# batmanlab/Mammo-CLIP

Hardware: AMD Instinct MI355X
Metric: image-text pairs/s (whole node), EN-B5+BioClinicalBERT contrastive pre-training step (higher is better)
Workload: dtype bf16; 1 GPU; cfg4: efficientnet-b5 + BioClinicalBERT(BERT-base), 1024 pairs/GPU (2 views + 2 reports each), 1520x912 images, 256-token reports, breast_clip loss, AdamW; fwd+loss+bwd+optimizer; dropout/drop-connect on; global_batch=1024, parallelism=dp1 x 32 micro-batches, keep_graphs=7, recompute=0, keep_recompute=2, stat_tapes=True, streams=3

## Files before the change

include/mammoclip_hip.h:

```cpp
#ifndef MAMMOCLIP_HIP_H
#define MAMMOCLIP_HIP_H
#include <stdint.h>
#ifdef __cplusplus
extern "C" {
#endif

typedef uint16_t mc_bf16;

const char* mc_last_error(void);
int mc_version(void);
int mc_storage_is_f16(void);

typedef struct mc_gemm_args {
    const mc_bf16* A;
    const mc_bf16* B;
    void* C;
    long long M, K;
    int N;
    long long lda, ldb, ldc;
    int a_kmajor, b_kmajor;
    int c_f32, c_atomic;
    int splits;
    int batch, nb2;
    long long sA1, sA2, sB1, sB2, sC1, sC2;
// ... 154 lines not shown

typedef struct mc_bnact_args {
    const mc_bf16* x;
    long long n_img, hw;
    int c;
    const float* scale;
    const float* shift;
    int act;
    const float* rowscale;
    const mc_bf16* res;
    mc_bf16* out;
    float* pooled;
    const mc_bf16* g;
    const float* mul;
    const float* add;
    float add_scale;
    const float* mean;
    const float* invstd;
    float* partials;
    const float* coef;
    mc_bf16* dx;
    float* dgate;
    float* split_ws;
} mc_bnact_args;
int mc_bnact_rows(const mc_bnact_args* args);
int mc_bnact_img_splits(const mc_bnact_args* args);
int mc_bnact_apply(const mc_bnact_args* args, void* stream);
int mc_bnact_pool(const mc_bnact_args* args, void* stream);
int mc_bnact_bwd_reduce(const mc_bnact_args* args, void* stream);
int mc_bnact_bwd_apply(const mc_bnact_args* args, void* stream);
int mc_bnact_se_dgate(const mc_bnact_args* args, void* stream);
int mc_bnact_se_sums(const mc_bnact_args* args, void* stream);
int mc_bn_partials_from_se_sums(const float* sums, const float* gate, const float* dpooled, float add_scale,
                                long long n_img, int c, float* partials, void* stream);
int mc_bn_bwd_finalize(const float* partials, int rows, int c, double count, const float* gamma,
                       const float* mean, const float* invstd, float* dgamma, float* dbeta, float* coef,
                       void* stream);

int mc_bn_fold_prepare(const float* we, const float* coef, const float* xtx, const float* colsum_x, double rows, int n,
                       int k, mc_bf16* w1t, mc_bf16* wb, mc_bf16* sxx, void* stream);
int mc_bn_fold_cvec(const float* gt, const float* we, const float* coef, const float* dbeta, const float* colsum_x,
                    double rows, int n, int k, mc_bf16* gtb, float* cvec, void* stream);
int mc_bn_fold_wgrad(const float* t1, const float* wx, const float* coef, const float* dbeta, const float* colsum_x,
                     double rows, int n, int k, float* dwe, void* stream);
int mc_bn_gram_partials(const mc_bf16* w, int ldw, const float* xtx, const float* colsum_x, double rows, int n, int k,
                        float* partials, void* stream);

int mc_colsum_rows(long long m, int c);
int mc_colsum_bf16(const mc_bf16* x, long long m, int c, long long ld, float* partials, float* out,
                   int accumulate, void* stream);

int mc_se_fwd(const float* pooled, const float* w1, const float* b1, const float* w2, const float* b2,
              int n, int c, int cs, float* gate, float* ws , void* stream);
int mc_se_bwd(const float* pooled, const float* gate, const float* dgate, const float* w1, const float* b1,
              const float* w2, const float* b2, int n, int c, int cs, float* dpooled, float* dw1, float* db1,
              float* dw2, float* db2, float* ws, void* stream);

int mc_dropout_f32(const float* x, float* y, long long n, float p, unsigned long long seed,
                   unsigned int stream_id, void* stream);

int mc_bert_embed_fwd(const long long* ids, const long long* tt, const float* word, const float* pos,
                      const float* type, const float* gamma, const float* beta, float eps, int b, int t,
                      int h, float p, unsigned long long seed, unsigned int stream_id, mc_bf16* y,
                      float* mean, float* rstd, void* stream);
int mc_bert_embed_bwd(const mc_bf16* dy, const long long* ids, const long long* tt, const float* word,
                      const float* pos, const float* type, const float* gamma, const float* mean,
                      const float* rstd, int b, int t, int h, float p, unsigned long long seed,
                      unsigned int stream_id, float* dword, float* dpos, float* dtype, float* dgamma,
                      float* dbeta, void* stream);
// ... 106 lines not shown
```

mammo_clip_amd/breastclip/model/modules/efficientnet_custom.py:

```python
import math
from collections import namedtuple
from typing import List, Optional

import os

import torch
from torch import nn

from .... import ops

BN_MOMENTUM = 0.01
BN_EPS = 1e-3

VALID_MODELS = tuple(f"efficientnet-b{i}" for i in range(9)) + ("efficientnet-l2",)

_COEFFS = {
    "efficientnet-b0": (1.0, 1.0, 224, 0.2), "efficientnet-b1": (1.0, 1.1, 240, 0.2),
    "efficientnet-b2": (1.1, 1.2, 260, 0.3), "efficientnet-b3": (1.2, 1.4, 300, 0.3),
    "efficientnet-b4": (1.4, 1.8, 380, 0.4), "efficientnet-b5": (1.6, 2.2, 456, 0.4),
    "efficientnet-b6": (1.8, 2.6, 528, 0.5), "efficientnet-b7": (2.0, 3.1, 600, 0.5),
    "efficientnet-b8": (2.2, 3.6, 672, 0.5), "efficientnet-l2": (4.3, 5.3, 800, 0.5),
}
_STAGES = ((1, 3, 1, 1, 32, 16), (2, 3, 2, 6, 16, 24), (2, 5, 2, 6, 24, 40), (3, 3, 2, 6, 40, 80),
           (3, 5, 1, 6, 80, 112), (4, 5, 2, 6, 112, 192), (1, 3, 1, 6, 192, 320))
# ... 175 lines not shown
        n, h, wd, oh, ow, c0 = ctx.geo
        mod = ctx.mod
        link = ctx.link
        if link is not None:
            de, dgamma, dbeta = ops.bnact_bwd(e, n, oh * ow, c0, ctx.st, mod._bn0.weight, 0, g=dy.contiguous(), partials=link.part)
            link.part = None
        else:
            de, dgamma, dbeta = ops.bnact_bwd(e, n, oh * ow, c0, ctx.st, mod._bn0.weight, 1, g=dy.contiguous())
        l, r, t, b = mod.stem_pad
        patches = ops.stem_im2col(x, l, t, oh, ow)
        dw = ops.linear_wgrad(de, patches)
        gw, gg, gb = ops.deliver_param_grads((mod._conv_stem.weight, mod._bn0.weight, mod._bn0.bias),
                                             (dw[:, :27].reshape(c0, 3, 3, 3), dgamma, dbeta))
        return (None, gw, gg, gb, None) + ((None,) if link is not None else ())


class _StemLink:
    __slots__ = ("st", "part")

    def __init__(self):
        self.st, self.part = None, None


def _expand_conv(pl, x, we, stats=True):
    if pl.fp8_expand:
        return ops.linear_fwd_fp8(x, we, stats=True)
    return _conv_stats(ops.linear_fwd, pl.training, x, we, stats=stats)


def _depthwise(blk, pl, x, e, we, wkkc, pro0, stats=True):
    if pl.xdw:
        return _conv_stats(ops.mbconv_xdw_fwd, pl.training, x, we, pro0, wkkc, *pl.dw, stats=stats)
    return _conv_stats(ops.dwconv_fwd, pl.training, e if blk.args.expand != 1 else x, wkkc, *pl.dw, stats=stats, pro=pro0)


def _project_conv(pl, d, act1, st1, gate, wp, stats=True):
    ohw = pl.oh * pl.ow
    if pl.fp8_project:
        wg = ops.gate_weights(wp, gate)
        return ops.linear_fwd_fp8(act1, wg, stats=True, batch_w=(pl.n, ohw))
    src, pro = (act1, (None, None, gate, ohw)) if pl.keep_act else (d, (st1.scale, st1.shift, gate, ohw))
    return _conv_stats(ops.linear_fwd, pl.training, src, wp, stats=stats, pro=pro)


class _MBConvFn(torch.autograd.Function):

    @staticmethod
    def forward(ctx, x, rowscale, blk, n, h, w, recording, link, *params):
        a = blk.args
        pl = blk.plan(n, h, w, recording)
        training, ohw = pl.training, pl.oh * pl.ow
        wkkc = blk.w_taps()
        e = we = st0 = gram = None
        if a.expand != 1:
            we = blk.w_expand()
            if pl.xdw:
                if training and _replaying():
                    part0, gram = None, _TAPE.get()
                elif training:
                    part0, gram = ops.bn_gram_partials(x, we, n * h * w)
                    if _TAPE is not None:
                        _TAPE.put(gram)
                else:
                    part0 = None
            else:
                e, part0 = _expand_conv(pl, x, we)
            st0 = _bn_stats(part0, n * h * w, blk._bn0, training)
            pro0 = (st0.scale, st0.shift)
        else:
            pro0 = (link.st.scale, link.st.shift) if link is not None else None
        d, part1 = _depthwise(blk, pl, x, e, we, wkkc, pro0)
        st1 = _bn_stats(part1, n * ohw, blk._bn1, training)
        if pl.keep_act:
            pooled, act1 = ops.bnact_pool(d, n, ohw, a.cexp, st1.scale, st1.shift, 1, keep_act=True)
        elif training and _replaying():
            pooled, act1 = _TAPE.get(), None
        else:
            pooled, act1 = ops.bnact_pool(d, n, ohw, a.cexp, st1.scale, st1.shift, 1), None
            if training and _TAPE is not None:
                _TAPE.put(pooled)
        if training and _replaying():
            gate = _TAPE.get()
        else:
            gate = ops.se_fwd(pooled, blk._se_reduce.weight.view(a.cse, a.cexp), blk._se_reduce.bias,
                              blk._se_expand.weight.view(a.cexp, a.cse), blk._se_expand.bias)
            if training and _TAPE is not None:
                _TAPE.put(gate)
        wp = blk.w_project()
        p, part2 = _project_conv(pl, d, act1, st1, gate, wp)
        st2 = _bn_stats(part2, n * ohw, blk._bn2, training)
        y = ops.bnact_apply(p, n, ohw, a.cout, st2.scale, st2.shift, 0,
                            rowscale=rowscale if a.skip else None, res=x if a.skip else None)
        ctx.blk, ctx.plan, ctx.saved = blk, pl, dict(
            x=x, e=e if pl.store_e else None, d=d if pl.store_d else None, act1=act1 if pl.store_d else None,
            p=p if pl.store_p else None, we=we, wkkc=wkkc, wp=wp, pro0=pro0, link=link, st0=st0, st1=st1, st2=st2, gram=gram,
            pooled=pooled, gate=gate, efree=pl.efree, rowscale=rowscale if a.skip else None)
        return y

    @staticmethod
    def backward(ctx, dy):
        blk, pl, sv = ctx.blk, ctx.plan, ctx.saved
        a = blk.args
        n, h, w, oh, ow = pl.n, pl.h, pl.w, pl.oh, pl.ow
        hw, ohw = h * w, oh * ow
        k, s, l, t = a.k, a.s, a.pad[0], a.pad[2]
        dy = dy.contiguous()
        x, e, d, p, act1, link, pro0 = sv["x"], sv["e"], sv["d"], sv["p"], sv["act1"], sv["link"], sv["pro0"]
        st0, st1, st2, gate, pooled = sv["st0"], sv["st1"], sv["st2"], sv["gate"], sv["pooled"]
        if a.expand != 1 and e is None and not (pl.efree or pl.efree_s2):
            e = _expand_conv(pl, x, sv["we"], stats=False)[0]
        if d is None:
            d = _depthwise(blk, pl, x, e, sv["we"], sv["wkkc"], pro0, stats=False)[0]
            if pl.keep_act:
                act1 = ops.bnact_pool(d, n, ohw, a.cexp, st1.scale, st1.shift, 1, keep_act=True)[1]
        if p is None:
# ... 50 lines not shown
            da0 = ops.dwconv_bwd_data(dd, sv["wkkc"], *pl.dw, w_kkc_flipped=wflip)
            del dd
        if a.expand != 1:
            if de is not None:
                we_t = blk.w_expand(transposed=True)
                if pl.xbwd:
                    dx, dwe = ops.xbwd_rows(de, x, we_t, residual=dy if a.skip else None)
                else:
                    dx = ops.linear_dgrad(de, sv["we"], residual=dy if a.skip else None, w_t=we_t)
                    dwe = ops.linear_wgrad(de, x)
            grads["_expand_conv.weight"] = dwe.view(a.cexp, a.cin, 1, 1)
            grads["_bn0.weight"], grads["_bn0.bias"] = dg0, db0
        else:
            dx = da0
            if a.skip:
                dx = ops.bnact_apply(da0, n, hw, a.cin, blk._ones, blk._zeros, 0, res=dy)
        grads["_depthwise_conv.weight"] = ops.transpose_f32(dwdw).view(a.cexp, 1, k, k)
        grads["_bn1.weight"], grads["_bn1.bias"] = dg1, db1n
        grads["_se_reduce.weight"], grads["_se_reduce.bias"] = dw1.view(a.cse, a.cexp, 1, 1), db1
        grads["_se_expand.weight"], grads["_se_expand.bias"] = dw2.view(a.cexp, a.cse, 1, 1), dbse2
        grads["_project_conv.weight"] = dwp.view(a.cout, a.cexp, 1, 1)
        grads["_bn2.weight"], grads["_bn2.bias"] = dg2, db2
        ctx.saved = None
        return (dx, None, None, None, None, None, None, None) + ops.deliver_param_grads(blk._params(), [grads[nm] for nm in blk._param_names])


class _HeadFn(torch.autograd.Function):

    @staticmethod
    def forward(ctx, x, w, gamma, beta, mod, n, h, wd):
        cin, cout = w.shape[1], w.shape[0]
        wb = ops.cast_bf16(w.view(cout, cin))
        if mod.fp8 and cin % 16 == 0:
            e, part = ops.linear_fwd_fp8(x, wb, stats=True)
        else:
            e, part = _conv_stats(ops.linear_fwd, mod.training, x, wb)
        st = _bn_stats(part, n * h * wd, mod._bn1, mod.training)
        pooled = ops.bnact_pool(e, n, h * wd, cout, st.scale, st.shift, 1)
        ctx.mod, ctx.st, ctx.geo = mod, st, (n, h, wd, cin, cout)
        ctx.save_for_backward(x, e, wb)
        mod._head_cache = (e, st, n, h, wd, cout)
        return pooled

    @staticmethod
    def backward(ctx, dpooled):
        x, e, wb = ctx.saved_tensors
        n, h, wd, cin, cout = ctx.geo
# ... 114 lines not shown
    def w_taps(self, flipped=False):
        v = self._depthwise_conv.weight.view(self.args.cexp, self.args.k * self.args.k)
        return ops.flipped_taps_f32(v) if flipped else ops.transpose_f32(v, cache=True)

    def w_project(self, transposed=False):
        v = self._project_conv.weight.view(self.args.cout, self.args.cexp)
        return ops.cast_transpose_bf16(v) if transposed else ops.cast_bf16(v)

    def _params(self):
        cached = self.__dict__.get("_plist")
        if cached is not None:
            ps, slots = cached
            for p_, (d_, k_) in zip(ps, slots):
                if d_.get(k_) is not p_:
                    cached = None
                    break
        if cached is None:
            slots = [(m._parameters, k) for m in self.modules() for k, v in m._parameters.items() if v is not None]
            ps = [d_[k_] for d_, k_ in slots]
            assert len(ps) == len(self._param_names)
            self.__dict__["_plist"] = (ps, slots)
        return ps

    def forward(self, inputs, n, h, w, rowscale=None, link=None):
        return _MBConvFn.apply(inputs, rowscale, self, n, h, w, torch.is_grad_enabled(), link, *self._params())


class EfficientNet(nn.Module):

    def __init__(self, blocks_args: List[BlockArgs] = None, global_params: GlobalParams = None):
        super().__init__()
        assert isinstance(blocks_args, list) and len(blocks_args) > 0
        self._global_params, self._blocks_args = global_params, blocks_args
        gp = global_params
        size = (gp.image_size, gp.image_size) if isinstance(gp.image_size, int) else tuple(gp.image_size)
        c0 = _scaled_width(32, gp)
        self._conv_stem = _Conv(3, c0, 3, 2)
        self._bn0 = _BN(c0)
        self.stem_pad = _static_pad(size, 3, 2)
        size = _down(size, 2)
        self._blocks = nn.ModuleList([])
        for ba in blocks_args:
            ba = ba._replace(input_filters=_scaled_width(ba.input_filters, gp),
                             output_filters=_scaled_width(ba.output_filters, gp),
                             num_repeat=_scaled_depth(ba.num_repeat, gp))
            s = ba.stride if isinstance(ba.stride, int) else ba.stride[0]
            self._blocks.append(MBConvBlock(ba, gp, size, idx=len(self._blocks)))
            size = _down(size, s)
# ... 62 lines not shown

    def xdw_reforward_modes(self):
        changed = []
        for blk in self._blocks:
            if blk.recompute == 0 and blk.xdw_capable():
                changed.append((blk, blk.recompute))
                blk.recompute = 1
        return changed

    def set_swish(self, memory_efficient=True):
        """No-op: the swish is always the fused, recompute-in-backward form."""

    def stem_geo(self, n, h, w):
        l, r, t, b = self.stem_pad
        return n, _out_extent(h, t, b, 3, 2), _out_extent(w, l, r, 3, 2)

    def _stem(self, x):
        b0 = self._blocks[0].args
        link = _StemLink() if (LINK_STEM and b0.expand == 1 and not b0.skip and b0.s == 1) else None
        args = (x, self._conv_stem.weight, self._bn0.weight, self._bn0.bias, self)
        y = _StemFn.apply(*args, link) if link is not None else _StemFn.apply(*args)
        return y, link, self.stem_geo(x.shape[0], *x.shape[2:])

    def _drop_connect_scales(self, n, device, seed):
        rate = self._global_params.drop_connect_rate
        out = []
        nb = len(self._blocks)
        for i, blk in enumerate(self._blocks):
            p = rate * float(i) / nb if rate else 0.0
            if not (self.training and p > 0.0 and blk.args.skip):
                out.append(None)
                continue
            out.append(ops.dropout_f32(self._ones_b.expand(n).contiguous(), p, seed, 1000 + i))
        return out

    def _features_nhwc(self, inputs):
        if not inputs.is_cuda:
            raise RuntimeError("mammo_clip_amd.EfficientNet runs only on a HIP device (no CPU fallback)")
        x = inputs if isinstance(inputs, ops.RawImages) or inputs.dtype == torch.float32 else inputs.float()
        seed = self.rng.next()
        self._last_seed = seed
        counters = [] if self.training else None
        bns = self._bn_layers if counters is not None else ()
        for bn in bns:
            bn.defer_count = counters
        try:
            y, link, (n, h, w) = self._stem(x)
            scales = self._drop_connect_scales(n, x.device, seed)
            for blk, rs in zip(self._blocks, scales):
                y = blk(y, n, h, w, rs, link if blk.args.idx == 0 else None)
                n, h, w = blk.out_geo(n, h, w)
        finally:
            for bn in bns:
                bn.defer_count = None
        self._pending_counters = counters
        return y, n, h, w

    def warm_weight_images(self, backward: bool):
        for blk in self._blocks:
            if blk.args.expand != 1:
                blk.w_expand()
                if backward:
                    blk.w_expand(transposed=True)
            blk.w_taps()
            if backward and blk.args.s == 1:
                blk.w_taps(flipped=True)
            blk.w_project()
            if backward:
                blk.w_project(transposed=True)
        cout, cin = self._conv_head.weight.shape[0], self._conv_head.weight.shape[1]
        ops.cast_bf16(self._conv_head.weight.view(cout, cin))
        if backward:
            ops.cast_transpose_bf16(self._conv_head.weight.view(cout, cin))

# ... 25 lines not shown
            if torch.is_tensor(t_) and t_.is_cuda:
                t_.record_stream(side)
        seeds = [self.rng.next(), self.rng.next()]
        training = self.training
        counters = [[], []] if training else [None, None]
        bns = self._bn_layers if training else ()
        defer = None

        def chain(i):
            global _BN_DEFER
            torch.cuda.set_stream(side if i else main)
            for bn in bns:
                bn.defer_count = counters[i]
            _BN_DEFER = defer if i else None

        ys, scales, links = [None, None], [None, None], [None, None]
        try:
            torch.cuda.set_stream(side)
            defer = _BNDefer(self) if training else None
            for i in (0, 1):
                chain(i)
                ys[i], links[i], (n, h, w) = self._stem(xs[i])
                scales[i] = self._drop_connect_scales(n, xs[i].device, seeds[i])
            for bi, blk in enumerate(self._blocks):
                for i in (0, 1):
                    chain(i)
                    ys[i] = blk(ys[i], n, h, w, scales[i][bi], links[i] if bi == 0 else None)
                n, h, w = blk.out_geo(n, h, w)
            pooled = [None, None]
            for i in (0, 1):
                chain(i)
                pooled[i] = _HeadFn.apply(ys[i], self._conv_head.weight, self._bn1.weight, self._bn1.bias, self, n, h, w)
                if training and self._dropout_p > 0.0:
                    pooled[i] = _DropoutFn.apply(pooled[i], self._dropout_p, seeds[i], 999)
        finally:
            torch.cuda.set_stream(main)
            for bn in bns:
                bn.defer_count = None
            _BN_DEFER = None
        self._last_seed = seeds[1]
        main.wait_stream(side)
        if defer is not None:
            defer.apply()
        with torch.no_grad():
            for c in counters:
                if c:
                    torch._foreach_add_(c, 1)
        pooled[1].record_stream(main)
        return pooled[0], pooled[1]

    def _flush_counters(self):
# ... 30 lines not shown
```

mammo_clip_amd/csrc/bnact.hip:

```cpp
#include "common_hip.h"
#include "../../include/mammoclip_hip.h"

namespace {

__host__ __device__ inline int rowmap_width(int cv, int cbase, bool split_small) {
    if (cbase > 0) return (cv - cbase) < 256 ? (cv - cbase) : 256;
    if (cv > 256) return 256;
    if (!split_small || cv * (256 / cv) * 10 >= 256 * 7) return cv;
    int a = 1;
    while (a * 2 <= cv) a *= 2;
    return a;
}

struct RowMap {
    int cv, cvp, rpb, rl, cl;
    bool split_small;
    __device__ RowMap(int c, bool split_small_ = false) {
        cv = c / 8;
        split_small = split_small_;
        set(0);
    }
    __device__ void set(int cbase) {
        cvp = rowmap_width(cv, cbase, split_small);
        rpb = 256 / cvp;
// ... 52 lines not shown
    if (var < 0.0) var = 0.0;
    float is = (float)(1.0 / sqrt(var + (double)eps));
    mean[i] = (float)m;
    invstd[i] = is;
    float sc = gamma[i] * is;
    scale[i] = sc;
    shift[i] = beta[i] - (float)m * sc;
    if (update) {
        double unbiased = count > 1.0 ? var * count / (count - 1.0) : var;
        rmean[i] = (1.f - momentum) * rmean[i] + momentum * (float)m;
        rvar[i] = (1.f - momentum) * rvar[i] + momentum * (float)unbiased;
    }
}

__global__ void bn_eval_coeffs_k(const float* gamma, const float* beta, const float* rm, const float* rv, float eps,
                                 int c, float* scale, float* shift) {
    int i = blockIdx.x * blockDim.x + threadIdx.x;
    if (i >= c) return;
    float sc = gamma[i] / sqrtf(rv[i] + eps);
    scale[i] = sc;
    shift[i] = beta[i] - rm[i] * sc;
}

__global__ __launch_bounds__(256) void bnact_apply_k(const mc_bnact_args p) {
    const int cvn = p.c / 8;
    const long long total = p.n_img * p.hw * cvn;
    for (long long i = (long long)blockIdx.x * 256 + threadIdx.x; i < total; i += (long long)gridDim.x * 256) {
        int cv = (int)(i % cvn);
        long long pix = i / cvn;
        float f[8], s[8], t[8];
        unpack8(nt_load16(p.x + pix * p.c + cv * 8), f);
        load8f(p.scale + cv * 8, s);
        load8f(p.shift + cv * 8, t);
        float rs = p.rowscale ? p.rowscale[pix / p.hw] : 1.f;
        if (p.act == 1) bn_silu8(f, s, t);
        else {
#pragma unroll
            for (int q = 0; q < 8; ++q) f[q] = f[q] * s[q] + t[q];
        }
#pragma unroll
        for (int q = 0; q < 8; ++q) f[q] *= rs;
        if (p.res) {
            float r[8];
            unpack8(nt_load16(p.res + pix * p.c + cv * 8), r);
#pragma unroll
            for (int q = 0; q < 8; ++q) f[q] += r[q];
        }
        *reinterpret_cast<uint4*>(p.out + pix * p.c + cv * 8) = pack8(f);
    }
}

template <int MODE>
__global__ __launch_bounds__(256) void bnact_img_reduce_k(const mc_bnact_args p) {
    RowMap rm(p.c, MODE == 0);
    __shared__ float red[256 * 8];
    __shared__ float tmp[256];
    const long long img = blockIdx.x;
    const bf16_t* xb = p.x + img * p.hw * p.c;
    const bf16_t* gb = (MODE == 1) ? p.g + img * p.hw * p.c : nullptr;
    float* dst = (MODE == 0 ? p.pooled : p.dgate) + img * p.c;
    const float post = (MODE == 0) ? 1.0f / (float)p.hw : 1.0f;
    for (int cbase = 0; cbase < rm.cv; cbase += rm.cvp) {
        rm.set(cbase);
        int v = cbase + rm.cl;
        float acc[8];
#pragma unroll
        for (int q = 0; q < 8; ++q) acc[q] = 0.f;
        if (rm.rl < rm.rpb && v < rm.cv) {
            float s[8], t[8];
            load8f(p.scale + v * 8, s);
            load8f(p.shift + v * 8, t);
// ... 457 lines not shown
                       gamma, beta, running_mean, running_var, momentum, eps, update_running, mean, invstd, scale, shift);
    MC_LAUNCH_CHECK();
    return MC_OK;
}
extern "C" int mc_bn_eval_coeffs(const float* gamma, const float* beta, const float* running_mean,
                                 const float* running_var, float eps, int c, float* scale, float* shift, void* stream) {
    MC_CHECK(gamma && beta && running_mean && running_var && scale && shift && c > 0, "bn_eval_coeffs: bad args");
    hipLaunchKernelGGL(bn_eval_coeffs_k, dim3(mc_div_up(c, 128)), dim3(128), 0, (hipStream_t)stream, gamma, beta,
                       running_mean, running_var, eps, c, scale, shift);
    MC_LAUNCH_CHECK();
    return MC_OK;
}
static int bwd_grid_x(const mc_bnact_args& p) {
    int cv = p.c / 8;
    int cvp = rowmap_width(cv, 0, false);
    int rpb = 256 / (cvp > 0 ? cvp : 1);
    long long per = (p.hw + (long long)rpb * 32 - 1) / ((long long)rpb * 32);
    long long cap = 4096 / (p.n_img > 0 ? p.n_img : 1);
    if (cap < 1) cap = 1;
    long long gx = per < cap ? per : cap;
    return (int)(gx < 1 ? 1 : gx);
}
extern "C" int mc_bnact_rows(const mc_bnact_args* a) { return (int)(bwd_grid_x(*a) * a->n_img); }
extern "C" int mc_bnact_apply(const mc_bnact_args* a, void* stream) {
    const mc_bnact_args& p = *a;
    if (int e = check_bnact(p)) return e;
    MC_CHECK(p.out, "bnact_apply: null out");
    hipLaunchKernelGGL(bnact_apply_k, dim3(stream_blocks(p.n_img * p.hw * (p.c / 8))), dim3(256), 0, (hipStream_t)stream, p);
    MC_LAUNCH_CHECK();
    return MC_OK;
}
__global__ __launch_bounds__(256) void split_sum_k(const float* __restrict__ ws, float* __restrict__ out, long long n, int splits) {
    __shared__ float sh[4][64];
    const int el = threadIdx.x & 63, pl = threadIdx.x >> 6;
    const long long i = (long long)blockIdx.x * 64 + el;
    float s = 0.f;
    if (i < n) {
        int k = pl;
        for (; k + 12 < splits; k += 16) {
            const float a = ws[(long long)k * n + i], b = ws[(long long)(k + 4) * n + i];
            const float c = ws[(long long)(k + 8) * n + i], d = ws[(long long)(k + 12) * n + i];
            s += a; s += b; s += c; s += d;
        }
        for (; k < splits; k += 4) s += ws[(long long)k * n + i];
    }
    sh[pl][el] = s;
    __syncthreads();
    if (pl == 0 && i < n) out[i] = ((sh[0][el] + sh[1][el]) + sh[2][el]) + sh[3][el];
}
static int img_splits(const mc_bnact_args& p, long long target = 2048) {
// ... 126 lines not shown
```

mammo_clip_amd/csrc/bnfold.hip:

```cpp
#include "common_hip.h"
#include "../../include/mammoclip_hip.h"

namespace {

#ifdef MC_F16
#define MC_FOLD_ROWS(rows) (rows)
#else
#define MC_FOLD_ROWS(rows) 1.0
#endif
__global__ void fold_prepare_k(const float* __restrict__ we, const float* __restrict__ coef, const float* __restrict__ xtx,
                               const float* __restrict__ cs, double rows, int n, int k, bf16_t* __restrict__ w1t,
                               bf16_t* __restrict__ wb, bf16_t* __restrict__ sxx) {
    const long long nk = (long long)n * k, total = nk + (long long)k * k;
    for (long long idx = (long long)blockIdx.x * 256 + threadIdx.x; idx < total; idx += (long long)gridDim.x * 256) {
        if (idx < nk) {
            const int i = (int)(idx / k), j = (int)(idx % k);
            const float w = we[idx];
            w1t[(long long)j * n + i] = f2bf(w * coef[i]);
            wb[idx] = f2bf((float)((double)(w * coef[n + i]) * MC_FOLD_ROWS(rows)));
        } else {
            const long long r = idx - nk;
            const int i = (int)(r / k), j = (int)(r % k);
            sxx[r] = f2bf((float)(((double)xtx[r] - (double)cs[i] * (double)cs[j] / rows) / MC_FOLD_ROWS(rows)));
        }
// ... 43 lines not shown
    for (int idx = threadIdx.x; idx < k * k; idx += 256) {
        const int i = idx / k, j = idx - i * k;
        const double sij = (double)xtx[idx] - (double)cs[i] * (double)cs[j] / rows;
        q += (double)bf2f(wc[i]) * sij * (double)bf2f(wc[j]);
    }
    __shared__ double red[2][256];
    red[0][threadIdx.x] = s; red[1][threadIdx.x] = q;
    __syncthreads();
    for (int st = 128; st > 0; st >>= 1) {
        if (threadIdx.x < st) { red[0][threadIdx.x] += red[0][threadIdx.x + st]; red[1][threadIdx.x] += red[1][threadIdx.x + st]; }
        __syncthreads();
    }
    if (threadIdx.x == 0) {
        const double sum = red[0][0];
        double sq = red[1][0];
        if (sq < 0.0) sq = 0.0;
        sq += sum * sum / rows;
        const float s_hi = (float)sum, q_hi = (float)sq;
        part[c] = s_hi; part[n + c] = q_hi;
        part[2 * n + c] = (float)(sum - (double)s_hi); part[3 * n + c] = (float)(sq - (double)q_hi);
    }
}

}

extern "C" int mc_bn_gram_partials(const mc_bf16* w, int ldw, const float* xtx, const float* colsum_x, double rows, int n, int k,
                                   float* partials, void* stream) {
    MC_CHECK(w && xtx && colsum_x && partials && n > 0 && k > 0 && ldw >= k && rows > 0, "bn_gram_partials: bad args");
    hipLaunchKernelGGL(gram_partials_k, dim3(n), dim3(256), 0, (hipStream_t)stream, (const bf16_t*)w, ldw, xtx, colsum_x, rows, n, k,
                       partials);
    MC_LAUNCH_CHECK();
    return MC_OK;
}

extern "C" int mc_bn_fold_prepare(const float* we, const float* coef, const float* xtx, const float* colsum_x, double rows,
                                  int n, int k, mc_bf16* w1t, mc_bf16* wb, mc_bf16* sxx, void* stream) {
    MC_CHECK(we && coef && xtx && colsum_x && w1t && wb && sxx && n > 0 && k > 0 && rows > 0, "bn_fold_prepare: bad args");
    const long long total = (long long)n * k + (long long)k * k;
    hipLaunchKernelGGL(fold_prepare_k, dim3((unsigned)((total + 255) / 256 < 2048 ? (total + 255) / 256 : 2048)), dim3(256), 0,
                       (hipStream_t)stream, we, coef, xtx, colsum_x, rows, n, k, (bf16_t*)w1t, (bf16_t*)wb, (bf16_t*)sxx);
    MC_LAUNCH_CHECK();
    return MC_OK;
}

extern "C" int mc_bn_fold_cvec(const float* gt, const float* we, const float* coef, const float* dbeta,
                               const float* colsum_x, double rows, int n, int k, mc_bf16* gtb, float* cvec, void* stream) {
// ... 17 lines not shown
```

mammo_clip_amd/lib.py:

```python
import ctypes as C
import os

_HERE = os.path.dirname(os.path.abspath(__file__))
STORAGE = os.environ.get("MC_STORAGE", "bf16").lower()
if STORAGE not in ("bf16", "f16"):
    raise ValueError(f"MC_STORAGE must be 'bf16' or 'f16', got {STORAGE!r}")
LIB_PATH = os.path.join(_HERE, "lib", "libmammoclip_hip.so" if STORAGE == "bf16" else "libmammoclip_hip_f16.so")

P, LL, I, F, D, U, ULL = C.c_void_p, C.c_longlong, C.c_int, C.c_float, C.c_double, C.c_uint, C.c_ulonglong


class GemmArgs(C.Structure):
    _fields_ = [
        ("A", P), ("B", P), ("C", P),
        ("M", LL), ("K", LL), ("N", I),
        ("lda", LL), ("ldb", LL), ("ldc", LL),
        ("a_kmajor", I), ("b_kmajor", I),
        ("c_f32", I), ("c_atomic", I),
        ("splits", I),
        ("batch", I), ("nb2", I),
        ("sA1", LL), ("sA2", LL), ("sB1", LL), ("sB2", LL), ("sC1", LL), ("sC2", LL),
        ("bias", P), ("bias_stride1", LL),
        ("act", I),
        ("R", P), ("ldr", LL),
# ... 33 lines not shown
    ]


class DwconvArgs(C.Structure):
    _fields_ = [
        ("x", P), ("dy", P), ("out", P), ("w_kkc", P),
        ("n", I), ("h", I), ("w", I), ("c", I),
        ("k", I), ("stride", I), ("pad_l", I), ("pad_t", I), ("oh", I), ("ow", I),
        ("pro_scale", P), ("pro_shift", P), ("stat_partials", P),
        ("epi_x", P), ("epi_scale", P), ("epi_shift", P), ("epi_mean", P), ("epi_invstd", P),
        ("dw_out", P), ("stat_rows", I),
        ("xw", P), ("cin", I),
    ]


class BnactArgs(C.Structure):
    _fields_ = [
        ("x", P), ("n_img", LL), ("hw", LL), ("c", I),
        ("scale", P), ("shift", P), ("act", I),
        ("rowscale", P), ("res", P), ("out", P),
        ("pooled", P),
        ("g", P), ("mul", P), ("add", P), ("add_scale", F), ("mean", P), ("invstd", P),
        ("partials", P), ("coef", P), ("dx", P), ("dgate", P), ("split_ws", P),
    ]


class AdamwTensor(C.Structure):
    _fields_ = [("param", P), ("grad", P), ("exp_avg", P), ("exp_avg_sq", P), ("numel", LL), ("bf16_image", P)]


_SIGS = {
    "mc_version": ([], I),
    "mc_storage_is_f16": ([], I),
    "mc_adamw_step": ([C.POINTER(AdamwTensor), I, D, D, D, D, D, LL, P], I),
    "mc_grads_unscale": ([C.POINTER(AdamwTensor), I, F, P, P], I),
    "mc_grads_unscale_dev": ([C.POINTER(AdamwTensor), I, P, P, P], I),
    "mc_adamw_step_ls": ([C.POINTER(AdamwTensor), I, D, D, D, D, D, LL, P, P, P], I),
    "mc_loss_scale_update": ([P, P, D, D, I, I, P], I),
    "mc_grad_norm_partials": ([C.POINTER(AdamwTensor), I], LL),
    "mc_grad_norm": ([C.POINTER(AdamwTensor), I, P, LL, F, P, P], I),
    "mc_grads_unscale_norm_dev": ([C.POINTER(AdamwTensor), I, P, P, P, LL, F, P, P], I),
    "mc_grads_scale_dev": ([C.POINTER(AdamwTensor), I, P, P], I),
    "mc_adamw_step_clip": ([C.POINTER(AdamwTensor), I, D, D, D, D, D, LL, P, P, P, P], I),
    "mc_gemm_bf16": ([C.POINTER(GemmArgs), P], I),
    "mc_gemm_stat_rows": ([C.POINTER(GemmArgs)], I),
    "mc_gemm_tile_config": ([C.POINTER(GemmArgs)], I),
# ... 20 lines not shown
    "mc_stem_weight_prep": ([P, P, I, P], I),
    "mc_stem_im2col": ([P, LL, LL, LL, LL, I, I, I, I, I, I, I, P, P], I),
    "mc_image_minmax_u8": ([P, LL, LL, I, P, P], I),
    "mc_gate_weights_bf16": ([P, P, I, I, I, P, P], I),
    "mc_stem_im2col_u8": ([P, LL, LL, LL, LL, P, F, F, I, I, I, I, I, I, I, P, P], I),
    "mc_dwconv_stat_rows": ([C.POINTER(DwconvArgs)], I),
    "mc_dwconv_bwd_data_stat_rows": ([C.POINTER(DwconvArgs)], I),
    "mc_dwconv_fwd": ([C.POINTER(DwconvArgs), P], I),
    "mc_dwconv_bwd_data": ([C.POINTER(DwconvArgs), P], I),
    "mc_dwconv_bwd_data_xw_supported": ([C.POINTER(DwconvArgs)], I),
    "mc_dwconv_bwd_data_plan": ([C.POINTER(DwconvArgs), C.POINTER(C.c_int)], I),
    "mc_dwconv_bwd_data_xw_preferred": ([C.POINTER(DwconvArgs)], I),
    "mc_dwconv_bwd_weight": ([C.POINTER(DwconvArgs), P], I),
    "mc_dwconv_set_lane_mode": ([I], I),
    "mc_dwconv_lane_supported": ([C.POINTER(DwconvArgs)], I),
    "mc_dwconv_bwd_fused_supported": ([C.POINTER(DwconvArgs)], I),
    "mc_dwconv_bwd_fused_preferred": ([C.POINTER(DwconvArgs)], I),
    "mc_dwconv_bwd_fused_stat_rows": ([C.POINTER(DwconvArgs)], I),
    "mc_dwconv_bwd_fused": ([C.POINTER(DwconvArgs), P], I),
    "mc_mbconv_xdw_supported": ([C.POINTER(DwconvArgs)], I),
    "mc_mbconv_xdw_stat_rows": ([C.POINTER(DwconvArgs)], I),
    "mc_mbconv_xdw_fwd": ([C.POINTER(DwconvArgs), P], I),
    "mc_bn_gram_partials": ([P, I, P, P, D, I, I, P, P], I),
    "mc_bn_finalize": ([P, I, I, D, P, P, P, P, F, F, I, P, P, P, P, P], I),
    "mc_bn_eval_coeffs": ([P, P, P, P, F, I, P, P, P], I),
    "mc_bnact_rows": ([C.POINTER(BnactArgs)], I),
    "mc_bnact_img_splits": ([C.POINTER(BnactArgs)], I),
    "mc_bnact_apply": ([C.POINTER(BnactArgs), P], I),
    "mc_bnact_pool": ([C.POINTER(BnactArgs), P], I),
    "mc_bnact_bwd_reduce": ([C.POINTER(BnactArgs), P], I),
    "mc_bnact_bwd_apply": ([C.POINTER(BnactArgs), P], I),
    "mc_bnact_se_dgate": ([C.POINTER(BnactArgs), P], I),
    "mc_bnact_se_sums": ([C.POINTER(BnactArgs), P], I),
    "mc_bn_partials_from_se_sums": ([P, P, P, F, LL, I, P, P], I),
    "mc_bn_bwd_finalize": ([P, I, I, D, P, P, P, P, P, P, P], I),
    "mc_colsum_rows": ([LL, I], I),
    "mc_colsum_bf16": ([P, LL, I, LL, P, P, I, P], I),
    "mc_se_fwd": ([P, P, P, P, P, I, I, I, P, P, P], I),
    "mc_se_bwd": ([P, P, P, P, P, P, P, I, I, I, P, P, P, P, P, P, P], I),
    "mc_dropout_f32": ([P, P, LL, F, ULL, U, P], I),
    "mc_bert_embed_fwd": ([P, P, P, P, P, P, P, F, I, I, I, F, ULL, U, P, P, P, P], I),
    "mc_bert_embed_bwd": ([P, P, P, P, P, P, P, P, P, I, I, I, F, ULL, U, P, P, P, P, P, P], I),
    "mc_add_ln_fwd": ([P, P, P, P, F, LL, I, F, ULL, U, P, P, P, P], I),
    "mc_add_ln_bwd": ([P, P, P, P, P, P, LL, I, F, ULL, U, P, P, P, P, P], I),
    "mc_softmax_fwd": ([P, LL, I, F, ULL, U, P, P, P], I),
    "mc_softmax_bwd": ([P, P, LL, I, F, ULL, U, F, P, P], I),
    "mc_bn_fold_prepare": ([P, P, P, P, D, I, I, P, P, P, P], I),
    "mc_bn_fold_cvec": ([P, P, P, P, P, D, I, I, P, P, P], I),
    "mc_bn_fold_wgrad": ([P, P, P, P, P, D, I, I, P, P], I),
# ... 117 lines not shown
```

mammo_clip_amd/ops.py:

```python
import ctypes as C
import math
import os

import weakref

import torch

from . import lib as L

BF16 = torch.bfloat16 if L.STORAGE == "bf16" else torch.float16


def _p(t):
    return None if t is None else t.data_ptr()


_RAW_STREAM = getattr(torch._C, "_cuda_getCurrentRawStream", None)
_GET_DEV = getattr(torch._C, "_cuda_getDevice", None)


def _st():
    if _RAW_STREAM is None or _GET_DEV is None:
        return torch.cuda.current_stream().cuda_stream
    return _RAW_STREAM(_GET_DEV())
# ... 653 lines not shown
        a = _dw_args(n, h, w, c, k, stride, pad_l, pad_t, oh, ow)
        a.cin = cin
        hit = _XDW_OK[key] = bool(L.load().mc_mbconv_xdw_supported(C.byref(a)))
    return hit


def mbconv_xdw_fwd(x, we, pro, w_kkc, n, h, w, c, k, stride, pad_l, pad_t, oh, ow, stats=False):
    cin = x.shape[1]
    assert we.shape == (c, cin) and we.is_contiguous() and x.is_contiguous()
    a = _dw_args(n, h, w, c, k, stride, pad_l, pad_t, oh, ow)
    y = empty((n * oh * ow, c), BF16, x)
    a.x, a.out, a.w_kkc, a.xw, a.cin = _p(x), _p(y), _p(w_kkc), _p(we), cin
    a.pro_scale, a.pro_shift = _p(pro[0]), _p(pro[1])
    part = None
    if stats:
        rows = L.load().mc_mbconv_xdw_stat_rows(C.byref(a))
        part = empty((rows, 2, c), torch.float32, x)
        a.stat_partials, a.stat_rows = _p(part), rows
    _note(2 * n * (cin * h * w + c * oh * ow) + 2 * c * cin, 2 * n * c * (oh * ow * k * k + h * w * cin))
    L.call("mc_mbconv_xdw_fwd", C.byref(a), _st(), kind=f"k{k}s{stride}")
    return (y, part) if stats else y


def bn_gram_partials(x, we, rows):
    c, cin = we.shape
    xtx = linear_wgrad(x, x, tag="_xtx")
    cs = colsum(x)
    part = empty((2, 2, c), torch.float32, x)
    L.call("mc_bn_gram_partials", _p(we), we.stride(0), _p(xtx), _p(cs), float(rows), c, cin, _p(part), _st())
    return part, (xtx, cs)


def _dwconv_bwd_weight_impl(x, dy, n, h, w, c, k, stride, pad_l, pad_t, oh, ow, pro=None):
    a = _dw_args(n, h, w, c, k, stride, pad_l, pad_t, oh, ow)
    dw = torch.zeros((k * k, c), dtype=torch.float32, device=x.device)
    a.x, a.dy, a.out = _p(x), _p(dy), _p(dw)
    if pro is not None:
        a.pro_scale, a.pro_shift = _p(pro[0]), _p(pro[1])
    _note(2 * n * c * (h * w + oh * ow), 2 * n * c * oh * ow * k * k)
    L.call("mc_dwconv_bwd_weight", C.byref(a), _st(), kind=f"k{k}s{stride}")
    return dw


class BNStats:
    __slots__ = ("mean", "invstd", "scale", "shift", "count")


def bn_finalize(partials, count, gamma, beta, running_mean, running_var, momentum, eps, update_running):
    rows, _, c = partials.shape
    buf = empty((4, c), torch.float32, partials)
    L.call("mc_bn_finalize", _p(partials), rows, c, float(count), _p(gamma), _p(beta), _p(running_mean),
           _p(running_var), momentum, eps, int(update_running), _p(buf[0]), _p(buf[1]), _p(buf[2]), _p(buf[3]), _st())
    s = BNStats()
    s.mean, s.invstd, s.scale, s.shift, s.count = buf[0], buf[1], buf[2], buf[3], float(count)
    return s


def bn_eval_coeffs(gamma, beta, running_mean, running_var, eps):
    c = gamma.shape[0]
    buf = empty((4, c), torch.float32, gamma)
    L.call("mc_bn_eval_coeffs", _p(gamma), _p(beta), _p(running_mean), _p(running_var), eps, c, _p(buf[2]), _p(buf[3]), _st())
    s = BNStats()
    s.mean, s.invstd, s.scale, s.shift, s.count = None, None, buf[2], buf[3], 0.0
    return s


def _bnact(x, n_img, hw, c, scale, shift, act):
    a = L.BnactArgs()
    a.x, a.n_img, a.hw, a.c = _p(x), n_img, hw, c
    a.scale, a.shift, a.act = _p(scale), _p(shift), act
    return a


def bnact_apply(x, n_img, hw, c, scale, shift, act, rowscale=None, res=None):
    a = _bnact(x, n_img, hw, c, scale, shift, act)
    out = empty((n_img * hw, c), BF16, x)
    a.rowscale, a.res, a.out = _p(rowscale), _p(res), _p(out)
    _note(2 * n_img * hw * c * (3 if res is not None else 2))
    L.call("mc_bnact_apply", C.byref(a), _st())
    return out


def _split_ws(a, x, n_img, c, planes=1):
    sp = L.load().mc_bnact_img_splits(C.byref(a))
    if sp <= 1:
        return None
    ws = empty((sp, planes, n_img, c), torch.float32, x)
    a.split_ws = _p(ws)
    return ws


def bnact_pool(x, n_img, hw, c, scale, shift, act, keep_act=False):
    a = _bnact(x, n_img, hw, c, scale, shift, act)
    pooled = empty((n_img, c), torch.float32, x)
    a.pooled = _p(pooled)
    y = None
    if keep_act:
        y = empty((n_img * hw, c), BF16, x)
        a.out = _p(y)
    ws = _split_ws(a, x, n_img, c)
    _note((4 if keep_act else 2) * n_img * hw * c)
    L.call("mc_bnact_pool", C.byref(a), _st())
    return (pooled, y) if keep_act else pooled
# ... 683 lines not shown
```

Baseline: 125.3 image-text pairs/s.

## Fuse next block's Gram matrix and column sums into the BN-apply epilogue

When the next MBConv block takes the xdw path, which needs X^T X and colsum(X) of its input for BN statistics, the current block's bnact_apply now computes these in the same pass with an MFMA-based Gram epilogue. The result is passed to the next block through a link object. This removes a separate re-read of the activation (the linear_wgrad xtx GEMM plus the colsum kernel) for narrow channel counts (c <= 64). It adds a new kernel whose per-block partials need an extra combine launch and workspace, and the Gram matrix is now accumulated from bf16-rounded outputs.

After: 126.4 image-text pairs/s, median of 6. No clear change (+0.8%).

```diff
diff --git a/include/mammoclip_hip.h b/include/mammoclip_hip.h
--- a/include/mammoclip_hip.h
+++ b/include/mammoclip_hip.h
@@ -200,8 +200,12 @@
     mc_bf16* dx;
     float* dgate;
     float* split_ws;
+    float* gram_ws;
+    float* gram_xtx;
+    float* gram_colsum;
 } mc_bnact_args;
 int mc_bnact_rows(const mc_bnact_args* args);
+int mc_bnact_gram_parts(const mc_bnact_args* args);
 int mc_bnact_img_splits(const mc_bnact_args* args);
 int mc_bnact_apply(const mc_bnact_args* args, void* stream);
 int mc_bnact_pool(const mc_bnact_args* args, void* stream);
@@ -223,6 +227,7 @@
                      double rows, int n, int k, float* dwe, void* stream);
 int mc_bn_gram_partials(const mc_bf16* w, int ldw, const float* xtx, const float* colsum_x, double rows, int n, int k,
                         float* partials, void* stream);
+int mc_bn_gram_combine(const float* ws, int parts, int k, float* xtx, float* colsum_x, void* stream);
 
 int mc_colsum_rows(long long m, int c);
 int mc_colsum_bf16(const mc_bf16* x, long long m, int c, long long ld, float* partials, float* out,
diff --git a/mammo_clip_amd/breastclip/model/modules/efficientnet_custom.py b/mammo_clip_amd/breastclip/model/modules/efficientnet_custom.py
--- a/mammo_clip_amd/breastclip/model/modules/efficientnet_custom.py
+++ b/mammo_clip_amd/breastclip/model/modules/efficientnet_custom.py
@@ -221,6 +221,18 @@
         self.st, self.part = None, None
 
 
+class _GramLink:
+    __slots__ = ("want", "pair", "ptr")
+
+    def __init__(self):
+        self.want, self.pair, self.ptr = False, None, 0
+
+    def take(self, x):
+        pair, ptr = self.pair, self.ptr
+        self.pair, self.ptr = None, 0
+        return pair if (pair is not None and ptr == x.data_ptr()) else None
+
+
 def _expand_conv(pl, x, we, stats=True):
     if pl.fp8_expand:
         return ops.linear_fwd_fp8(x, we, stats=True)
@@ -245,7 +257,7 @@
 class _MBConvFn(torch.autograd.Function):
 
     @staticmethod
-    def forward(ctx, x, rowscale, blk, n, h, w, recording, link, *params):
+    def forward(ctx, x, rowscale, blk, n, h, w, recording, link, glink, *params):
         a = blk.args
         pl = blk.plan(n, h, w, recording)
         training, ohw = pl.training, pl.oh * pl.ow
@@ -257,7 +269,7 @@
                 if training and _replaying():
                     part0, gram = None, _TAPE.get()
                 elif training:
-                    part0, gram = ops.bn_gram_partials(x, we, n * h * w)
+                    part0, gram = ops.bn_gram_partials(x, we, n * h * w, gram=glink.take(x) if glink is not None else None)
                     if _TAPE is not None:
                         _TAPE.put(gram)
                 else:
@@ -288,8 +300,12 @@
         wp = blk.w_project()
         p, part2 = _project_conv(pl, d, act1, st1, gate, wp)
         st2 = _bn_stats(part2, n * ohw, blk._bn2, training)
+        want = glink is not None and glink.want and training and not _replaying() and ops.bnact_gram_ok(a.cout)
         y = ops.bnact_apply(p, n, ohw, a.cout, st2.scale, st2.shift, 0,
-                            rowscale=rowscale if a.skip else None, res=x if a.skip else None)
+                            rowscale=rowscale if a.skip else None, res=x if a.skip else None, gram=want)
+        if want:
+            y, glink.pair = y
+            glink.ptr = y.data_ptr()
         ctx.blk, ctx.plan, ctx.saved = blk, pl, dict(
             x=x, e=e if pl.store_e else None, d=d if pl.store_d else None, act1=act1 if pl.store_d else None,
             p=p if pl.store_p else None, we=we, wkkc=wkkc, wp=wp, pro0=pro0, link=link, st0=st0, st1=st1, st2=st2, gram=gram,
@@ -386,7 +402,7 @@
         grads["_project_conv.weight"] = dwp.view(a.cout, a.cexp, 1, 1)
         grads["_bn2.weight"], grads["_bn2.bias"] = dg2, db2
         ctx.saved = None
-        return (dx, None, None, None, None, None, None, None) + ops.deliver_param_grads(blk._params(), [grads[nm] for nm in blk._param_names])
+        return (dx, None, None, None, None, None, None, None, None) + ops.deliver_param_grads(blk._params(), [grads[nm] for nm in blk._param_names])
 
 
 class _HeadFn(torch.autograd.Function):
@@ -547,8 +563,12 @@
             self.__dict__["_plist"] = (ps, slots)
         return ps
 
-    def forward(self, inputs, n, h, w, rowscale=None, link=None):
-        return _MBConvFn.apply(inputs, rowscale, self, n, h, w, torch.is_grad_enabled(), link, *self._params())
+    def forward(self, inputs, n, h, w, rowscale=None, link=None, glink=None):
+        return _MBConvFn.apply(inputs, rowscale, self, n, h, w, torch.is_grad_enabled(), link, glink, *self._params())
+
+    def wants_gram(self, n, h, w):
+        return (self.training and self.xdw_capable() and ops.bnact_gram_ok(self.args.cin)
+                and self.plan(n, h, w, torch.is_grad_enabled()).xdw)
 
 
 class EfficientNet(nn.Module):
@@ -657,6 +677,13 @@
         y = _StemFn.apply(*args, link) if link is not None else _StemFn.apply(*args)
         return y, link, self.stem_geo(x.shape[0], *x.shape[2:])
 
+    def _gram_link(self):
+        if not (ops.GRAM_PRODUCER and self.training) or _replaying():
+            return None
+        if any(blk._forward_hooks or blk._forward_pre_hooks for blk in self._blocks):
+            return None
+        return _GramLink()
+
     def _drop_connect_scales(self, n, device, seed):
         rate = self._global_params.drop_connect_rate
         out = []
@@ -682,9 +709,13 @@
         try:
             y, link, (n, h, w) = self._stem(x)
             scales = self._drop_connect_scales(n, x.device, seed)
-            for blk, rs in zip(self._blocks, scales):
-                y = blk(y, n, h, w, rs, link if blk.args.idx == 0 else None)
-                n, h, w = blk.out_geo(n, h, w)
+            glink = self._gram_link()
+            for bi, (blk, rs) in enumerate(zip(self._blocks, scales)):
+                geo = blk.out_geo(n, h, w)
+                if glink is not None:
+                    glink.want = bi + 1 < len(self._blocks) and self._blocks[bi + 1].wants_gram(*geo)
+                y = blk(y, n, h, w, rs, link if blk.args.idx == 0 else None, glink)
+                n, h, w = geo
         finally:
             for bn in bns:
                 bn.defer_count = None
@@ -756,11 +787,16 @@
                 chain(i)
                 ys[i], links[i], (n, h, w) = self._stem(xs[i])
                 scales[i] = self._drop_connect_scales(n, xs[i].device, seeds[i])
+            glinks = [self._gram_link(), self._gram_link()]
             for bi, blk in enumerate(self._blocks):
+                geo = blk.out_geo(n, h, w)
+                want = glinks[0] is not None and bi + 1 < len(self._blocks) and self._blocks[bi + 1].wants_gram(*geo)
                 for i in (0, 1):
                     chain(i)
-                    ys[i] = blk(ys[i], n, h, w, scales[i][bi], links[i] if bi == 0 else None)
-                n, h, w = blk.out_geo(n, h, w)
+                    if glinks[i] is not None:
+                        glinks[i].want = want
+                    ys[i] = blk(ys[i], n, h, w, scales[i][bi], links[i] if bi == 0 else None, glinks[i])
+                n, h, w = geo
             pooled = [None, None]
             for i in (0, 1):
                 chain(i)
diff --git a/mammo_clip_amd/csrc/bnact.hip b/mammo_clip_amd/csrc/bnact.hip
--- a/mammo_clip_amd/csrc/bnact.hip
+++ b/mammo_clip_amd/csrc/bnact.hip
@@ -98,31 +98,160 @@
     shift[i] = beta[i] - rm[i] * sc;
 }
 
+__device__ __forceinline__ uint4 bnact_apply8(const uint4& xv, const float* s, const float* t, int act, float rs, bool has_res,
+                                              const uint4& rv) {
+    float f[8];
+    unpack8(xv, f);
+    if (act == 1) bn_silu8(f, s, t);
+    else {
+#pragma unroll
+        for (int q = 0; q < 8; ++q) f[q] = __builtin_fmaf(f[q], s[q], t[q]);
+    }
+#pragma unroll
+    for (int q = 0; q < 8; ++q) {
+        f[q] *= rs;
+        asm volatile("" : "+v"(f[q]));
+    }
+    if (has_res) {
+        float r[8];
+        unpack8(rv, r);
+#pragma unroll
+        for (int q = 0; q < 8; ++q) f[q] += r[q];
+    }
+    return pack8(f);
+}
+
 __global__ __launch_bounds__(256) void bnact_apply_k(const mc_bnact_args p) {
     const int cvn = p.c / 8;
     const long long total = p.n_img * p.hw * cvn;
     for (long long i = (long long)blockIdx.x * 256 + threadIdx.x; i < total; i += (long long)gridDim.x * 256) {
         int cv = (int)(i % cvn);
         long long pix = i / cvn;
-        float f[8], s[8], t[8];
-        unpack8(nt_load16(p.x + pix * p.c + cv * 8), f);
+        float s[8], t[8];
+        const uint4 xv = nt_load16(p.x + pix * p.c + cv * 8);
         load8f(p.scale + cv * 8, s);
         load8f(p.shift + cv * 8, t);
         float rs = p.rowscale ? p.rowscale[pix / p.hw] : 1.f;
-        if (p.act == 1) bn_silu8(f, s, t);
-        else {
-#pragma unroll
-            for (int q = 0; q < 8; ++q) f[q] = f[q] * s[q] + t[q];
-        }
-#pragma unroll
-        for (int q = 0; q < 8; ++q) f[q] *= rs;
-        if (p.res) {
-            float r[8];
-            unpack8(nt_load16(p.res + pix * p.c + cv * 8), r);
-#pragma unroll
-            for (int q = 0; q < 8; ++q) f[q] += r[q];
-        }
-        *reinterpret_cast<uint4*>(p.out + pix * p.c + cv * 8) = pack8(f);
+        const uint4 rv = p.res ? nt_load16(p.res + pix * p.c + cv * 8) : make_uint4(0u, 0u, 0u, 0u);
+        *reinterpret_cast<uint4*>(p.out + pix * p.c + cv * 8) = bnact_apply8(xv, s, t, p.act, rs, p.res != nullptr, rv);
+    }
+}
+
+typedef __attribute__((ext_vector_type(4))) short s4_t;
+typedef __attribute__((address_space(3))) s4_t lds_s4_t;
+__device__ __forceinline__ bf16x8_t tr_frag(const unsigned char* tile, int rs, int row0, int col0, int lane) {
+    const int g = lane >> 4, i = lane & 15;
+    const unsigned char* a = tile + (size_t)(row0 + g * 8 + (i >> 2)) * rs + (col0 + (i & 3) * 4) * 2;
+    s4_t lo = __builtin_amdgcn_ds_read_tr16_b64_v4i16((lds_s4_t*)(a));
+    s4_t hi = __builtin_amdgcn_ds_read_tr16_b64_v4i16((lds_s4_t*)(a + 4 * rs));
+    typedef __attribute__((ext_vector_type(8))) short s8_t;
+    s8_t v = {lo[0], lo[1], lo[2], lo[3], hi[0], hi[1], hi[2], hi[3]};
+    return __builtin_bit_cast(bf16x8_t, v);
+}
+
+constexpr int GRAM_WROWS = 64;
+constexpr int GRAM_SROWS = 4 * GRAM_WROWS;
+constexpr int GRAM_MAX_PARTS = 512;
+
+template <int CV>
+__global__ __launch_bounds__(256, 2) void bnact_apply_gram_k(const mc_bnact_args p) {
+    constexpr int C = CV * 8, NF = (C + 15) / 16, RPW = 64 / CV, NP = (GRAM_WROWS + RPW - 1) / RPW, RS = C * 2;
+    __shared__ __attribute__((aligned(16))) unsigned char tile[4 * GRAM_WROWS * RS + 64];
+    __shared__ float red[256 * 8];
+    const int tid = threadIdx.x, lane = tid & 63, wave = tid >> 6;
+    const int rl = lane / CV, cl = lane - rl * CV;
+    const bool lane_on = rl < RPW;
+    const long long M = p.n_img * p.hw, nsteps = (M + GRAM_SROWS - 1) / GRAM_SROWS;
+    const bool has_res = p.res != nullptr;
+    unsigned char* wt = tile + wave * GRAM_WROWS * RS;
+    float s[8], t[8], cs[8];
+#pragma unroll
+    for (int q = 0; q < 8; ++q) { s[q] = 0.f; t[q] = 0.f; cs[q] = 0.f; }
+    if (lane_on) { load8f(p.scale + cl * 8, s); load8f(p.shift + cl * 8, t); }
+    f32x4_t acc[NF][NF];
+#pragma unroll
+    for (int i = 0; i < NF; ++i)
+#pragma unroll
+        for (int j = 0; j < NF; ++j) acc[i][j] = (f32x4_t){0.f, 0.f, 0.f, 0.f};
+
+    const uint4 z4 = make_uint4(0u, 0u, 0u, 0u);
+    uint4 xv[NP], rv[NP];
+    float rsv[NP];
+    auto load_step = [&](long long st) {
+        const long long row0 = st * GRAM_SROWS + wave * GRAM_WROWS;
+#pragma unroll
+        for (int u = 0; u < NP; ++u) {
+            const int r = u * RPW + rl;
+            const long long pix = row0 + r;
+            const bool ok = lane_on && r < GRAM_WROWS && pix < M;
+            xv[u] = ok ? nt_load16(p.x + pix * C + cl * 8) : z4;
+            rv[u] = (ok && has_res) ? nt_load16(p.res + pix * C + cl * 8) : z4;
+            rsv[u] = (ok && p.rowscale) ? p.rowscale[pix / p.hw] : 1.f;
+        }
+    };
+    long long st = blockIdx.x;
+    if (st < nsteps) load_step(st);
+    for (; st < nsteps; st += gridDim.x) {
+        const long long row0 = st * GRAM_SROWS + wave * GRAM_WROWS;
+#pragma unroll
+        for (int u = 0; u < NP; ++u) {
+            const int r = u * RPW + rl;
+            if (lane_on && r < GRAM_WROWS) {
+                const long long pix = row0 + r;
+                uint4 o = z4;
+                if (pix < M) {
+                    o = bnact_apply8(xv[u], s, t, p.act, rsv[u], has_res, rv[u]);
+                    *reinterpret_cast<uint4*>(p.out + pix * C + cl * 8) = o;
+                    float g[8];
+                    unpack8(o, g);
+#pragma unroll
+                    for (int q = 0; q < 8; ++q) cs[q] += g[q];
+                }
+                *reinterpret_cast<uint4*>(wt + r * RS + cl * 16) = o;
+            }
+        }
+        __syncthreads();
+        if (st + gridDim.x < nsteps) load_step(st + gridDim.x);
+#pragma unroll
+        for (int ks = 0; ks < GRAM_WROWS / 32; ++ks) {
+            bf16x8_t a[NF];
+#pragma unroll
+            for (int i = 0; i < NF; ++i) a[i] = tr_frag(wt, RS, ks * 32, i * 16, lane);
+#pragma unroll
+            for (int i = 0; i < NF; ++i)
+#pragma unroll
+                for (int j = 0; j < NF; ++j) acc[i][j] = MC_MFMA_16x16x32(a[i], a[j], acc[i][j], 0, 0, 0);
+        }
+        __syncthreads();
+    }
+    float* G = reinterpret_cast<float*>(tile);
+    for (int w = 0; w < 4; ++w) {
+        if (wave == w) {
+#pragma unroll
+            for (int i = 0; i < NF; ++i)
+#pragma unroll
+                for (int j = 0; j < NF; ++j) {
+                    const int k = j * 16 + (lane & 15);
+#pragma unroll
+                    for (int r = 0; r < 4; ++r) {
+                        const int n = i * 16 + (lane >> 4) * 4 + r;
+                        if (n < C && k < C) G[n * C + k] = w == 0 ? acc[i][j][r] : G[n * C + k] + acc[i][j][r];
+                    }
+                }
+        }
+        __syncthreads();
+    }
+#pragma unroll
+    for (int q = 0; q < 8; ++q) red[tid * 8 + q] = cs[q];
+    __syncthreads();
+    float* W = p.gram_ws + (long long)blockIdx.x * (C * (C + 1));
+    for (int e = tid; e < C * C; e += 256) W[e] = G[e];
+    if (tid < C) {
+        const int v = tid >> 3, q = tid & 7;
+        float sm = 0.f;
+        for (int w = 0; w < 4; ++w)
+            for (int r = 0; r < RPW; ++r) sm += red[(w * 64 + r * CV + v) * 8 + q];
+        W[C * C + tid] = sm;
     }
 }
 
@@ -626,10 +755,30 @@
     return (int)(gx < 1 ? 1 : gx);
 }
 extern "C" int mc_bnact_rows(const mc_bnact_args* a) { return (int)(bwd_grid_x(*a) * a->n_img); }
+extern "C" int mc_bnact_gram_parts(const mc_bnact_args* a) {
+    if (a->c <= 0 || a->c % 8 || a->c > 64 || a->n_img <= 0 || a->hw <= 0) return 0;
+    const long long steps = (a->n_img * a->hw + GRAM_SROWS - 1) / GRAM_SROWS;
+    return (int)(steps < GRAM_MAX_PARTS ? steps : GRAM_MAX_PARTS);
+}
 extern "C" int mc_bnact_apply(const mc_bnact_args* a, void* stream) {
     const mc_bnact_args& p = *a;
     if (int e = check_bnact(p)) return e;
     MC_CHECK(p.out, "bnact_apply: null out");
+    if (p.gram_ws || p.gram_xtx || p.gram_colsum) {
+        MC_CHECK(p.gram_ws && p.gram_xtx && p.gram_colsum, "bnact_apply: the Gram epilogue needs gram_ws, gram_xtx and gram_colsum");
+        const int parts = mc_bnact_gram_parts(a);
+        MC_CHECK(parts > 0, "bnact_apply: the Gram epilogue takes c <= 64 (see mc_bnact_gram_parts)");
+        MC_CHECK(mc_aligned16(p.out) && (!p.res || mc_aligned16(p.res)), "bnact_apply: out / res must be 16-byte aligned");
+        const dim3 grid(parts), block(256);
+        hipStream_t st = (hipStream_t)stream;
+        switch (p.c / 8) {
+#define GRAM_CASE(CV_) case CV_: hipLaunchKernelGGL((bnact_apply_gram_k<CV_>), grid, block, 0, st, p); break;
+            GRAM_CASE(1) GRAM_CASE(2) GRAM_CASE(3) GRAM_CASE(4) GRAM_CASE(5) GRAM_CASE(6) GRAM_CASE(7) GRAM_CASE(8)
+#undef GRAM_CASE
+        }
+        MC_LAUNCH_CHECK();
+        return mc_bn_gram_combine(p.gram_ws, parts, p.c, p.gram_xtx, p.gram_colsum, stream);
+    }
     hipLaunchKernelGGL(bnact_apply_k, dim3(stream_blocks(p.n_img * p.hw * (p.c / 8))), dim3(256), 0, (hipStream_t)stream, p);
     MC_LAUNCH_CHECK();
     return MC_OK;
diff --git a/mammo_clip_amd/csrc/bnfold.hip b/mammo_clip_amd/csrc/bnfold.hip
--- a/mammo_clip_amd/csrc/bnfold.hip
+++ b/mammo_clip_amd/csrc/bnfold.hip
@@ -89,6 +89,38 @@
     }
 }
 
+__global__ __launch_bounds__(256) void gram_combine_k(const float* __restrict__ ws, int parts, int k, float* __restrict__ xtx,
+                                                      float* __restrict__ cs) {
+    __shared__ double sh[16][17];
+    const int el = threadIdx.x & 15, pl = threadIdx.x >> 4;
+    const int n = k * (k + 1), i = blockIdx.x * 16 + el;
+    double s = 0.0;
+    if (i < n) {
+        int q = pl;
+        for (; q + 48 < parts; q += 64) {
+            const float a = ws[(long long)q * n + i], b = ws[(long long)(q + 16) * n + i];
+            const float c = ws[(long long)(q + 32) * n + i], d = ws[(long long)(q + 48) * n + i];
+            s += (double)a; s += (double)b; s += (double)c; s += (double)d;
+        }
+        for (; q < parts; q += 16) s += (double)ws[(long long)q * n + i];
+    }
+    sh[pl][el] = s;
+    __syncthreads();
+    if (pl != 0 || i >= n) return;
+    s = 0.0;
+    for (int q = 0; q < 16; ++q) s += sh[q][el];
+    if (i < k * k) xtx[i] = (float)s;
+    else cs[i - k * k] = (float)s;
+}
+
+}
+
+extern "C" int mc_bn_gram_combine(const float* ws, int parts, int k, float* xtx, float* colsum_x, void* stream) {
+    MC_CHECK(ws && xtx && colsum_x && parts > 0 && k > 0, "bn_gram_combine: bad args");
+    hipLaunchKernelGGL(gram_combine_k, dim3(mc_div_up((long long)k * (k + 1), 16)), dim3(256), 0, (hipStream_t)stream, ws, parts, k,
+                       xtx, colsum_x);
+    MC_LAUNCH_CHECK();
+    return MC_OK;
 }
 
 extern "C" int mc_bn_gram_partials(const mc_bf16* w, int ldw, const float* xtx, const float* colsum_x, double rows, int n, int k,
diff --git a/mammo_clip_amd/lib.py b/mammo_clip_amd/lib.py
--- a/mammo_clip_amd/lib.py
+++ b/mammo_clip_amd/lib.py
@@ -79,6 +79,7 @@
         ("pooled", P),
         ("g", P), ("mul", P), ("add", P), ("add_scale", F), ("mean", P), ("invstd", P),
         ("partials", P), ("coef", P), ("dx", P), ("dgate", P), ("split_ws", P),
+        ("gram_ws", P), ("gram_xtx", P), ("gram_colsum", P),
     ]
 
 
@@ -145,9 +146,11 @@
     "mc_mbconv_xdw_stat_rows": ([C.POINTER(DwconvArgs)], I),
     "mc_mbconv_xdw_fwd": ([C.POINTER(DwconvArgs), P], I),
     "mc_bn_gram_partials": ([P, I, P, P, D, I, I, P, P], I),
+    "mc_bn_gram_combine": ([P, I, I, P, P, P], I),
     "mc_bn_finalize": ([P, I, I, D, P, P, P, P, F, F, I, P, P, P, P, P], I),
     "mc_bn_eval_coeffs": ([P, P, P, P, F, I, P, P, P], I),
     "mc_bnact_rows": ([C.POINTER(BnactArgs)], I),
+    "mc_bnact_gram_parts": ([C.POINTER(BnactArgs)], I),
     "mc_bnact_img_splits": ([C.POINTER(BnactArgs)], I),
     "mc_bnact_apply": ([C.POINTER(BnactArgs), P], I),
     "mc_bnact_pool": ([C.POINTER(BnactArgs), P], I),
diff --git a/mammo_clip_amd/ops.py b/mammo_clip_amd/ops.py
--- a/mammo_clip_amd/ops.py
+++ b/mammo_clip_amd/ops.py
@@ -699,10 +699,20 @@
     return (y, part) if stats else y
 
 
-def bn_gram_partials(x, we, rows):
+GRAM_PRODUCER = os.environ.get("MC_GRAM_PRODUCER", "1") != "0"
+
+
+def bnact_gram_ok(c):
+    return GRAM_PRODUCER and c % 8 == 0 and 0 < c <= 64
+
+
+def bn_gram_partials(x, we, rows, gram=None):
     c, cin = we.shape
-    xtx = linear_wgrad(x, x, tag="_xtx")
-    cs = colsum(x)
+    if gram is not None:
+        xtx, cs = gram
+    else:
+        xtx = linear_wgrad(x, x, tag="_xtx")
+        cs = colsum(x)
     part = empty((2, 2, c), torch.float32, x)
     L.call("mc_bn_gram_partials", _p(we), we.stride(0), _p(xtx), _p(cs), float(rows), c, cin, _p(part), _st())
     return part, (xtx, cs)
@@ -749,13 +759,21 @@
     return a
 
 
-def bnact_apply(x, n_img, hw, c, scale, shift, act, rowscale=None, res=None):
+def bnact_apply(x, n_img, hw, c, scale, shift, act, rowscale=None, res=None, gram=False):
     a = _bnact(x, n_img, hw, c, scale, shift, act)
     out = empty((n_img * hw, c), BF16, x)
     a.rowscale, a.res, a.out = _p(rowscale), _p(res), _p(out)
+    pair = None
+    if gram:
+        parts = L.load().mc_bnact_gram_parts(C.byref(a))
+        if parts <= 0:
+            raise ValueError(f"bnact_apply: no Gram epilogue for c = {c}")
+        ws = empty((parts, c * (c + 1)), torch.float32, x)
+        pair = (empty((c, c), torch.float32, x), empty((c,), torch.float32, x))
+        a.gram_ws, a.gram_xtx, a.gram_colsum = _p(ws), _p(pair[0]), _p(pair[1])
     _note(2 * n_img * hw * c * (3 if res is not None else 2))
     L.call("mc_bnact_apply", C.byref(a), _st())
-    return out
+    return (out, pair) if gram else out
 
 
 def _split_ws(a, x, n_img, c, planes=1):
```
